# lucasnewman/f5-tts-mlx

Measured on AMD Instinct MI355X. Metric: mel_frames_per_sec, higher is better.
Workload: dtype f16 (IEEE-half MFMA operands, fp32 accumulate / residual stream / LayerNorm / softmax state; meets the 1e-3 gate); 1 GPU; BASELINE configs[1]: F5-TTS 335M, 32-point euler (=62 DiT forwards, CFG), batch 1/GPU x 10 s (N=937) utterances, hipGraph=True; f16 (IEEE half) MFMA operands IN PLACE OF BASELINE's bf16 -- same width and MFMA rate, three more significand bits; plain bf16 fails the 1e-3 parity gate, see sub.b1_bf16; global_batch=1, seq_len=937, parallelism=dp1 (utterance sharding)

## Files before the change

### f5_tts_mlx_amd/csrc/gemm.hip

```cpp
#include "gemm.hpp"
#include "gemm_dev.hpp"
#include "rowops.hpp"
#include "lnrow.hpp"

namespace F5_NS {



template <int MB, int NB>
struct ResidPre {
    float x[MB][16][NB];
    float bias[NB], gate[NB];
    uint32_t keep[MB][4];
};
template <int MB, int NB>
__device__ __forceinline__ void resid_preload(const F5GemmArgs& p, ResidPre<MB, NB>& q, int row0, int colbase, int lane) {
    const int hi = lane >> 5, lcol = lane & 31;
    const bool keep_words = p.rowkeep != nullptr && (reinterpret_cast<uintptr_t>(p.rowkeep) & 3) == 0;
#pragma unroll
    for (int nb = 0; nb < NB; ++nb) {
        const int c = colbase + nb * 32 + lcol;
        const bool ok = c < p.N;
        q.bias[nb] = (p.bias != nullptr && ok) ? p.bias[c] : 0.0f;
        q.gate[nb] = ok ? p.gate[c] : 0.0f;
// ... 198 lines not shown
        pa[ks] = &smem[0][0] + swz_off(wm * (32 * MB) + frow, ks * 2 + fk);
        pb[ks] = &smem[0][0] + BMt * BK + swz_off(wn * (32 * NB) + frow, ks * 2 + fk);
    }
    static_assert(2 * (BMt + BNt) * BK * 2 <= 65536, "both buffers must be addressable by ds_read immediates");
#define REG_STEP(CUR, tt_)                                                                                    \
    {                                                                                                         \
        if ((tt_) + 1 < T) LOAD_TILE();                                                                       \
        _Pragma("unroll") for (int ks = 0; ks < 4; ++ks) {                                                    \
            op16x8 af[MB], bfr[NB];                                                                           \
            _Pragma("unroll") for (int mb = 0; mb < MB; ++mb)                                                 \
                af[mb] = *reinterpret_cast<const op16x8*>(pa[ks] + (CUR) * (BMt + BNt) * BK + mb * 32 * BK);  \
            _Pragma("unroll") for (int nb = 0; nb < NB; ++nb)                                                 \
                bfr[nb] = *reinterpret_cast<const op16x8*>(pb[ks] + (CUR) * (BMt + BNt) * BK + nb * 32 * BK); \
            _Pragma("unroll") for (int mb = 0; mb < MB; ++mb)                                                 \
                _Pragma("unroll") for (int nb = 0; nb < NB; ++nb)                                             \
                    acc[mb][nb] = F5_MFMA32(af[mb], bfr[nb], acc[mb][nb], 0, 0, 0); \
        }                                                                                                     \
        if ((tt_) + 1 < T) STORE_TILE(1 - (CUR));                                                             \
        __syncthreads();                                                                                      \
    }
    for (int tt = 0; tt < T; tt += 2) {
        REG_STEP(0, tt);
        if (tt + 1 < T) REG_STEP(1, tt + 1);
    }
#undef REG_STEP
#undef LOAD_TILE
#undef STORE_TILE

    if (small_tile_staged<EPI, NB>() && n0 + BNt <= p.N && (p.debug_flags & 2) == 0) {
        static_assert(!small_tile_staged<EPI, NB>() || 4 * small_tile_stage_elems<NB>() <= 2 * (BMt + BNt) * BK, "staging fits");
        __syncthreads();
        staged_epilogue_bf16<EPI, MB, NB>(p, acc, &smem[0][0] + wave * small_tile_stage_elems<NB>(), m0 + wm * (32 * MB),
                                          n0 + wn * (32 * NB), lane);
        return;
    }
    gemm_epilogue<EPI, MB, NB>(p, acc, m0, n0, wm, wn, lane);
    if (EPI == EPI_RESID_GATE && p.ln_counter) resid_ln_tail(p, tm, BMt, (p.N + BNt - 1) / BNt);
}

int f5_gemm_order = 0;
static bool gemm_mfast(const F5GemmArgs& a) {
    if (f5_gemm_order == 1) return false;
    if (f5_gemm_order == 2) return true;
    const size_t a_bytes = (size_t)(a.a_row_mod > 0 ? a.a_row_mod : a.M) * a.K * 2 * (a.nseg == 3 ? 2 : 1);
    return a_bytes <= (size_t)4 << 20;
}
static int ring_order(const F5GemmArgs& a, int tiles_m, int tiles_n) {
    const bool band_ok = tiles_n % 4 == 0 && tiles_n >= 8 && (long)tiles_m * tiles_n <= 512 && tiles_m >= 8;
    if ((f5_gemm_order == 3 || f5_gemm_order == 0) && band_ok) return tiles_n | (4 << 20);
    if (f5_gemm_order == 3) return tiles_n;
    return gemm_mfast(a) ? -tiles_m : tiles_n;
}

template <int EPI, int MB, int NB, int NST, int WM = 2, int WN = 2, int KS = 1, int ABL = 0, int FOLD = 0>
__global__ __launch_bounds__(64 * WM * WN * KS) void f5_gemm_ring_kernel(F5GemmArgs p, int tiles_n, int ntiles) {
    constexpr int NTG = 64 * WM * WN;
    constexpr int BMt = 32 * MB * WM, BNt = 32 * NB * WN;
    constexpr int NA = BMt * 8 / NTG, NW = BNt * 8 / NTG;
    static_assert(NA * NTG == BMt * 8 && NW * NTG == BNt * 8, "tile rows must divide over the threads");
    constexpr int G = NA + NW;
    constexpr int STAGE = (BMt + BNt) * BK;
    constexpr int RING = NST * STAGE;
    static_assert(KS * RING * 2 <= 160 * 1024, "LDS budget");
    __shared__ __attribute__((aligned(16))) op16_t smem_all[KS * RING];

    asm volatile("" ::"s"(p.A[0]), "s"(p.W[0]), "s"(p.lda), "s"(p.ldw), "s"(p.K), "s"(p.nseg), "s"(p.M), "s"(p.N), "s"(p.a_row_mod),
                 "s"(p.debug_flags), "s"(tiles_n), "s"(ntiles));
    if (EPI == EPI_RESID_GATE)
        asm volatile("" ::"s"(p.bias), "s"(p.out_f32), "s"(p.ldo), "s"(p.gate), "s"(p.rowkeep), "s"(p.ln_counter));
    const int bid = blockIdx.x;
    const int q = ntiles >> 3, r = ntiles & 7;
    const int xcd = bid & 7, idx = bid >> 3;
    const int tile = (xcd < r ? xcd * (q + 1) : r * (q + 1) + (xcd - r) * q) + idx;
    int tm, tn;
    if (tiles_n >= (1 << 20)) {
        const int band = tiles_n >> 20, tnn = tiles_n & ((1 << 20) - 1);
        const int per_band = band * (ntiles / tnn);
        const int b = tile / per_band, rem = tile - b * per_band;
        tm = rem / band;
        tn = b * band + (rem - tm * band);
    } else if (tiles_n > 0) {
        tm = tile / tiles_n;
        tn = tile - tm * tiles_n;
    } else {
        tn = tile / (-tiles_n);
        tm = tile - tn * (-tiles_n);
    }
    const int m0 = tm * BMt, n0 = tn * BNt;

    const int tid = threadIdx.x;
    const int lane = tid & 63;
    const int wave_all = __builtin_amdgcn_readfirstlane(tid >> 6);
    const int grp = wave_all / (WM * WN), wave = wave_all % (WM * WN);
    const int tg = tid - grp * NTG;
    const int wm = wave / WN, wn = wave % WN;
    op16_t* smem = smem_all + grp * RING;

    uint32_t a_src[NA], w_src[NW];
    int a_dst[NA], w_dst[NW];
#pragma unroll
    for (int i = 0; i < NA; ++i) {
        const int q_ = i * NTG + tg;
        const int row = q_ >> 3, chunk = (q_ & 7) ^ ((row >> 1) & 7);
        int gr = m0 + row;
        if (gr > p.M - 1) gr = p.M - 1;
        if (p.a_row_mod > 0) gr = gr % p.a_row_mod;
        a_src[i] = ((uint32_t)gr * (uint32_t)p.lda + chunk * 8) * 2u;
        a_dst[i] = (i * NTG + wave * 64) * 8;
    }
#pragma unroll
    for (int i = 0; i < NW; ++i) {
        const int q_ = i * NTG + tg;
        const int row = q_ >> 3, chunk = (q_ & 7) ^ ((row >> 1) & 7);
        w_src[i] = ((uint32_t)(n0 + row) * (uint32_t)p.ldw + chunk * 8) * 2u;
        w_dst[i] = BMt * BK + (i * NTG + wave * 64) * 8;
    }
    const int kt = p.K / BK;
    const int T = kt * p.nseg;
    const int Tg = T > grp ? (T - grp + KS - 1) / KS : 0;
    const int nit = (T + KS - 1) / KS;
    int is_seg = 0, is_k0 = grp * BK;
    while (is_k0 >= p.K) {
        is_k0 -= p.K;
        ++is_seg;
    }
#define RING_ISSUE(ST_)                                                                                      \
    {                                                                                                        \
        op16_t* st_ = smem + (ST_) * STAGE;                                                                  \
        const char* Ap_ = reinterpret_cast<const char*>((is_seg == 1) ? p.A[1] : p.A[0]);                    \
        const char* Wp_ = reinterpret_cast<const char*>((is_seg == 2) ? p.W[1] : p.W[0]);                    \
        const uint32_t kb_ = (uint32_t)is_k0 * 2u;                                                           \
        _Pragma("unroll") for (int i = 0; i < NA; ++i)                                                       \
            glds16(reinterpret_cast<const op16_t*>(Ap_ + (a_src[i] + kb_)), st_ + a_dst[i]);                 \
        _Pragma("unroll") for (int i = 0; i < NW; ++i)                                                       \
            glds16(reinterpret_cast<const op16_t*>(Wp_ + (w_src[i] + kb_)), st_ + w_dst[i]);                 \
        is_k0 += KS * BK;                                                                                    \
        while (is_k0 >= p.K) {                                          \
            is_k0 -= p.K;                                                                                    \
            ++is_seg;                                                                                        \
        }                                                                                                    \
    }

    f32x16 acc[MB][NB];
#pragma unroll
    for (int i = 0; i < MB; ++i)
#pragma unroll
        for (int j = 0; j < NB; ++j)
#pragma unroll
            for (int e = 0; e < 16; ++e) acc[i][j][e] = 0.0f;

    constexpr bool PRE_RESID = EPI == EPI_RESID_GATE && MB * NB <= 3;
    ResidPre<PRE_RESID ? MB : 1, PRE_RESID ? NB : 1> rpre;
    const bool use_pre = PRE_RESID && p.ln_counter == nullptr && (p.debug_flags & (8 | 256)) == 0;
    constexpr bool SHARE = KS > 1 && NB == KS && FOLD == 0 && EPI != EPI_QKV_ROPE;
    const bool share = SHARE && p.ln_counter == nullptr && (p.debug_flags & (8 | 256)) == 0;
    constexpr bool SHARE_PRE = SHARE && PRE_RESID;
    ResidPre<SHARE_PRE ? MB : 1, 1> rown;
    if constexpr (SHARE_PRE) {
        if (use_pre) resid_preload<MB, 1>(p, rown, m0 + wm * (32 * MB), n0 + wn * (32 * NB) + grp * 32, lane);
    }
    if (PRE_RESID && !SHARE_PRE && use_pre && grp == 0 && FOLD != 1)
        resid_preload<PRE_RESID ? MB : 1, PRE_RESID ? NB : 1>(p, rpre, m0 + wm * (32 * MB), n0 + wn * (32 * NB), lane);
    static_assert(FOLD == 0 || (FOLD == 1 && PRE_RESID && NB == 2) || (FOLD == 2 && EPI == EPI_GELU_TANH && NB == 2 && KS == 1 && WM * WN == 8),
                  "fold producer = the preloaded residual epilogue on 64-column wave tiles; fold consumer = the 8-wave GELU launch");
    ResidStagedPre<FOLD == 1 ? NB : 1> spre_p;
    if constexpr (FOLD == 1) {
        if (grp == 0) resid_staged_preload<NB>(p, spre_p, m0 + wm * (32 * MB), n0 + wn * (32 * NB), lane);
    }
    FoldPre fpre_c;
    fold_prefetch_clear(fpre_c);
    FoldStatsPre<8> spre_c;
    fold_stats_clear(spre_c);
    if constexpr (FOLD == 2) fold_stats_request_tr<1>(p, spre_c, fpre_c, m0 + wm * 32, n0 + wn * 64, lane);

#pragma unroll
    for (int st = 0; st < NST - 1; ++st)
        if (st < Tg) RING_ISSUE(st);

    const int frow = lane & 31;
    const int fk = lane >> 5;
    constexpr int SPS = 65536 / (STAGE * 2) < NST ? 65536 / (STAGE * 2) : NST;
    static_assert(SPS >= 1, "a stage must fit the ds_read offset field");
    constexpr int NSET = (NST + SPS - 1) / SPS;
    const op16_t* pa[NSET][4];
    const op16_t* pb[NSET][4];
#pragma unroll
    for (int w2 = 0; w2 < NSET; ++w2)
#pragma unroll
        for (int ks = 0; ks < 4; ++ks) {
            pa[w2][ks] = smem + w2 * SPS * STAGE + swz_off(wm * (32 * MB) + frow, ks * 2 + fk);
            pb[w2][ks] = smem + w2 * SPS * STAGE + BMt * BK + swz_off(wn * (32 * NB) + frow, ks * 2 + fk);
        }
    op16x8 abl_frag;
#pragma unroll
    for (int e = 0; e < 8; ++e) abl_frag[e] = (op16_t)0;
    if (ABL & 4) asm volatile("" : "+v"(abl_frag));
#define RING_STEP(ST_, jj_, TR_)                                                                                       \
    {                                                                                                               \
         \
        if ((jj_) + NST - 2 < Tg) {                                                                                 \
            if (NST == 4) asm volatile("s_waitcnt vmcnt(%0)" ::"n"(2 * G) : "memory");                              \
            else if (NST == 3) asm volatile("s_waitcnt vmcnt(%0)" ::"n"(G) : "memory");                             \
            else asm volatile("s_waitcnt vmcnt(0)" ::: "memory");                                                   \
        } else {                                                                                                    \
            asm volatile("s_waitcnt vmcnt(0)" ::: "memory");                                                        \
        }                                                                                                           \
        asm volatile("" ::: "memory");                                                                              \
        if (!(ABL & 8)) __builtin_amdgcn_s_barrier();                                                               \
        asm volatile("" ::: "memory");                                                                              \
        if (!(ABL & 1) && (jj_) + NST - 1 < Tg) RING_ISSUE(((ST_) + NST - 1) % NST);  \
        if (!(KS > 1 && (jj_) >= Tg)) {               \
            constexpr int W2 = (ST_) / SPS, SL = (ST_) % SPS;                                                        \
            _Pragma("unroll") for (int ks = 0; ks < 4; ++ks) {                                                      \
                op16x8 af[MB], bfr[NB];                                                                             \
                _Pragma("unroll") for (int mb = 0; mb < MB; ++mb)                                                   \
                    af[mb] = (ABL & 4) ? abl_frag : *reinterpret_cast<const op16x8*>(pa[W2][ks] + SL * STAGE + mb * 32 * BK); \
                _Pragma("unroll") for (int nb = 0; nb < NB; ++nb)                                                   \
                    bfr[nb] = (ABL & 4) ? abl_frag : *reinterpret_cast<const op16x8*>(pb[W2][ks] + SL * STAGE + nb * 32 * BK); \
                _Pragma("unroll") for (int mb = 0; mb < MB; ++mb)                                                   \
                    _Pragma("unroll") for (int nb = 0; nb < NB; ++nb) {                                             \
                        if (ABL & 2) asm volatile("" ::"v"(af[mb]), "v"(bfr[nb]));                                  \
                        else if (TR_) acc[mb][nb] = F5_MFMA32(bfr[nb], af[mb], acc[mb][nb], 0, 0, 0);               \
                        else acc[mb][nb] = F5_MFMA32(af[mb], bfr[nb], acc[mb][nb], 0, 0, 0);                        \
                    }                                                                                               \
            }                                                                                                       \
        }                                                                                                           \
    }
    if constexpr (FOLD == 2) {
        if (NST == 4) asm volatile("s_waitcnt vmcnt(%0)" ::"n"(2 * G) : "memory");
        else asm volatile("s_waitcnt vmcnt(0)" ::: "memory");
        fold_stats_pin(spre_c);
        fold_stats_finish_tr<1>(p, spre_c, fpre_c, m0 + wm * 32, lane, p.fold_mean_out != nullptr && n0 == 0 && wn == 0);
        fold_prefetch_pin(fpre_c);
        for (int jj = 0; jj < nit; jj += NST) {
            RING_STEP(0, jj, true);
            if (NST > 1 && jj + 1 < nit) RING_STEP(1 % NST, jj + 1, true);
            if (NST > 2 && jj + 2 < nit) RING_STEP(2 % NST, jj + 2, true);
            if (NST > 3 && jj + 3 < nit) RING_STEP(3 % NST, jj + 3, true);
        }
        __syncthreads();
        static_assert(FOLD != 2 || WM * WN * (small_tile_stage_elems<NB>() * 2 + 512) <= RING * 2, "staging + c1 | c2 scratch fit in the ring");
        float* fl = reinterpret_cast<float*>(smem_all + WM * WN * small_tile_stage_elems<NB>()) + wave * 128;
        staged_epilogue_tr<EPI, MB, NB, true>(p, acc, smem_all + wave * small_tile_stage_elems<NB>(), m0 + wm * (32 * MB), n0 + wn * (32 * NB), lane,
                                              fl, &fpre_c);
        return;
    }
    constexpr bool QKV_TR_OK = EPI == EPI_QKV_ROPE && (32 * NB) % 64 == 0 && (NB & (NB - 1)) == 0 && KS == 1 && WM * WN == 8;
    if (QKV_TR_OK && p.rope_g4k != nullptr && n0 + wn * (32 * NB) < 2 * p.dmodel) {
        for (int jj = 0; jj < nit; jj += NST) {
            RING_STEP(0, jj, true);
            if (NST > 1 && jj + 1 < nit) RING_STEP(1 % NST, jj + 1, true);
            if (NST > 2 && jj + 2 < nit) RING_STEP(2 % NST, jj + 2, true);
            if (NST > 3 && jj + 3 < nit) RING_STEP(3 % NST, jj + 3, true);
        }
        __syncthreads();
        staged_epilogue_tr_rope<MB, NB>(p, acc, smem_all + wave * small_tile_stage_elems<NB>(), m0 + wm * (32 * MB), n0 + wn * (32 * NB),
                                        lane);
        return;
    }
    for (int jj = 0; jj < nit; jj += NST) {
        RING_STEP(0, jj, false);
        if (NST > 1 && jj + 1 < nit) RING_STEP(1 % NST, jj + 1, false);
        if (NST > 2 && jj + 2 < nit) RING_STEP(2 % NST, jj + 2, false);
        if (NST > 3 && jj + 3 < nit) RING_STEP(3 % NST, jj + 3, false);
    }
#undef RING_STEP
#undef RING_ISSUE
    if constexpr (SHARE) {
        if (share) {
            constexpr int RED1 = MB * 16 * 64;
            constexpr int STG1 = small_tile_staged<EPI, 1>() ? small_tile_stage_elems<1>() : 0;
            constexpr int STGS = KS * WM * WN * STG1;
            static_assert(STGS * 2 + WM * WN * NB * (KS - 1) * RED1 * 4 <= KS * RING * 2, "staging + parked parts fit in the rings");
            float* red = reinterpret_cast<float*>(smem_all + STGS) + (size_t)wave * (NB * (KS - 1) * RED1) + lane;
            __syncthreads();
#pragma unroll
            for (int g = 0; g < KS; ++g)
                if (grp == g) {
#pragma unroll
                    for (int nb = 0; nb < NB; ++nb)
                        if (nb != g) {
                            float* dst = red + (nb * (KS - 1) + (g < nb ? g : g - 1)) * RED1;
#pragma unroll
                            for (int mb = 0; mb < MB; ++mb)
#pragma unroll
                                for (int e = 0; e < 16; ++e) dst[(mb * 16 + e) * 64] = acc[mb][nb][e];
                        }
                }
            __syncthreads();
            f32x16 own[MB][1];
#pragma unroll
            for (int g = 0; g < KS; ++g)
                if (grp == g) {
                    const float* src = red + g * (KS - 1) * RED1;
#pragma unroll
                    for (int mb = 0; mb < MB; ++mb)
#pragma unroll
                        for (int e = 0; e < 16; ++e) {
                            const float mine = acc[mb][g][e];
                            float s = g == 0 ? mine : src[(mb * 16 + e) * 64];
#pragma unroll
                            for (int h = 1; h < KS; ++h) s += h == g ? mine : src[(h < g ? h : h - 1) * RED1 + (mb * 16 + e) * 64];
                            own[mb][0][e] = s;
                        }
                }
            const int row0 = m0 + wm * (32 * MB), col0 = n0 + wn * (32 * NB) + grp * 32;
            if (small_tile_staged<EPI, NB>() && n0 + BNt <= p.N && (p.debug_flags & 2) == 0) {
                staged_epilogue_bf16<EPI, MB, 1>(p, own, smem_all + wave_all * STG1, row0, col0, lane);
                return;
            }
            if constexpr (SHARE_PRE) {
                if (use_pre) {
                    resid_epilogue_preloaded<MB, 1>(p, own, rown, row0, col0, lane);
                    return;
                }
            }
            gemm_epilogue<EPI, MB, 1>(p, own, m0, col0, wm, 0, lane);
            return;
        }
    }
    constexpr int STG = small_tile_staged<EPI, NB>() ? WM * WN * small_tile_stage_elems<NB>() : 0;
    if (KS > 1) {
        constexpr int RED = MB * NB * 16 * 64;
        static_assert(KS == 1 || STG * 2 + (KS - 1) * WM * WN * RED * 4 <= KS * RING * 2, "reduction area fits in the rings");
        float* red = reinterpret_cast<float*>(smem_all + STG);
        __syncthreads();
        if (grp > 0) {
            float* dst = red + (size_t)((grp - 1) * (WM * WN) + wave) * RED + lane;
#pragma unroll
            for (int mb = 0; mb < MB; ++mb)
#pragma unroll
                for (int nb = 0; nb < NB; ++nb)
#pragma unroll
                    for (int e = 0; e < 16; ++e) dst[((mb * NB + nb) * 16 + e) * 64] = acc[mb][nb][e];
        }
        __syncthreads();
        if (grp > 0) {
            if (EPI == EPI_RESID_GATE && p.ln_counter) resid_ln_tail(p, tm, BMt, (p.N + BNt - 1) / BNt);
            return;
        }
#pragma unroll
        for (int g = 1; g < KS; ++g) {
            const float* src = red + (size_t)((g - 1) * (WM * WN) + wave) * RED + lane;
#pragma unroll
            for (int mb = 0; mb < MB; ++mb)
#pragma unroll
                for (int nb = 0; nb < NB; ++nb)
#pragma unroll
                    for (int e = 0; e < 16; ++e) acc[mb][nb][e] += src[((mb * NB + nb) * 16 + e) * 64];
        }
    }
    if (small_tile_staged<EPI, NB>() && n0 + BNt <= p.N && (p.debug_flags & 2) == 0) {
        static_assert(STG <= RING, "staging fits");
        if (KS == 1) __syncthreads();
        staged_epilogue_bf16<EPI, MB, NB>(p, acc, smem_all + wave * small_tile_stage_elems<NB>(), m0 + wm * (32 * MB),
                                          n0 + wn * (32 * NB), lane);
        return;
    }
    if constexpr (FOLD == 1) {
        constexpr int RED_BYTES = (KS - 1) * WM * WN * MB * NB * 16 * 64 * 4;
        static_assert(RED_BYTES + WM * WN * 32 * (32 * NB + 4) * 4 <= KS * RING * 2, "staging behind the reduction area");
        float* stg = reinterpret_cast<float*>(reinterpret_cast<char*>(smem_all) + RED_BYTES) + wave * (32 * (32 * NB + 4));
        staged_epilogue_resid<MB, NB, true>(p, acc, stg, m0 + wm * (32 * MB), n0 + wn * (32 * NB), lane, &spre_p);
        return;
    }
    if constexpr (PRE_RESID) {
        if (use_pre) {
            resid_epilogue_preloaded<MB, NB>(p, acc, rpre, m0 + wm * (32 * MB), n0 + wn * (32 * NB), lane);
            return;
        }
    }
    gemm_epilogue<EPI, MB, NB>(p, acc, m0, n0, wm, wn, lane);
    if (EPI == EPI_RESID_GATE && p.ln_counter) resid_ln_tail(p, tm, BMt, (p.N + BNt - 1) / BNt);
}

template <int EPI, int MB, int NB, int NST, int WM = 2, int WN = 2, int KS = 1, int FOLD = 0>
static int launch_ring(const F5GemmArgs& a, hipStream_t stream) {
    const int tiles_m = f5_cdiv(a.M, 32 * MB * WM), tiles_n = f5_cdiv(a.N, 32 * NB * WN);
    const int ntiles = tiles_m * tiles_n;
    const int order = ring_order(a, tiles_m, tiles_n);
    hipLaunchKernelGGL((f5_gemm_ring_kernel<EPI, MB, NB, NST, WM, WN, KS, 0, FOLD>), dim3(ntiles), dim3(64 * WM * WN * KS), 0, stream, a, order, ntiles);
    F5_LAUNCH_CHECK();
    return 0;
}

template <int EPI, int MB, int NB>
static int launch_cfg(const F5GemmArgs& a, hipStream_t stream) {
    const int tiles_m = f5_cdiv(a.M, 64 * MB), tiles_n = f5_cdiv(a.N, 64 * NB);
    const int ntiles = tiles_m * tiles_n;
    hipLaunchKernelGGL((f5_gemm_kernel<EPI, MB, NB>), dim3(ntiles), dim3(256), 0, stream, a, tiles_n, ntiles);
    F5_LAUNCH_CHECK();
    return 0;
}

int f5_gemm_debug_flags = 0;

constexpr int FC_ROWS = 4, FC_MAXC = 8;
int f5_fold_consts_mfma = 1;
__global__ __launch_bounds__(256) void f5_fold_consts_kernel(const op16_t* __restrict__ w, int ldw, const float* __restrict__ bias,
                                                             const float* __restrict__ scale, const float* __restrict__ shift, size_t vec_stride,
                                                             int nvec, float* __restrict__ c1, float* __restrict__ c2, size_t out_stride, int N,
                                                             int K, F5FoldBatch bt) {
    w += (size_t)blockIdx.y * bt.w_stride;
    if (bias) bias += (size_t)blockIdx.y * bt.bias_stride;
    scale += (size_t)blockIdx.y * bt.mod_stride;
    shift += (size_t)blockIdx.y * bt.mod_stride;
    c1 += (size_t)blockIdx.y * bt.out_blk_stride;
    c2 += (size_t)blockIdx.y * bt.out_blk_stride;
    const int lane = threadIdx.x & 63, wave = threadIdx.x >> 6;
    const int n0 = (blockIdx.x * 4 + wave) * FC_ROWS;
    if (n0 >= N) return;
    const int nchunk = K >> 8;
    float wv[FC_ROWS][FC_MAXC][4];
#pragma unroll
    for (int r = 0; r < FC_ROWS; ++r) {
        const int n = n0 + r < N ? n0 + r : N - 1;
#pragma unroll
        for (int c = 0; c < FC_MAXC; ++c) {
            if (c < nchunk) {
                const op16x4 t = *reinterpret_cast<const op16x4*>(w + (size_t)n * ldw + c * 256 + lane * 4);
#pragma unroll
                for (int e = 0; e < 4; ++e) wv[r][c][e] = f5_op2f(t[e]);
            } else {
#pragma unroll
                for (int e = 0; e < 4; ++e) wv[r][c][e] = 0.0f;
            }
        }
    }
    for (int v = 0; v < nvec; ++v) {
        const float* sv = scale + (size_t)v * vec_stride;
        const float* bv = shift + (size_t)v * vec_stride;
        float a1[FC_ROWS], a2[FC_ROWS];
#pragma unroll
        for (int r = 0; r < FC_ROWS; ++r) a1[r] = a2[r] = 0.0f;
#pragma unroll
        for (int c = 0; c < FC_MAXC; ++c) {
            if (c < nchunk) {
                const f32x4 s4 = *reinterpret_cast<const f32x4*>(sv + c * 256 + lane * 4);
                const f32x4 b4 = *reinterpret_cast<const f32x4*>(bv + c * 256 + lane * 4);
#pragma unroll
                for (int r = 0; r < FC_ROWS; ++r)
#pragma unroll
                    for (int e = 0; e < 4; ++e) {
                        a1[r] += wv[r][c][e] * (1.0f + s4[e]);
                        a2[r] += wv[r][c][e] * b4[e];
                    }
            }
        }
#pragma unroll
        for (int r = 0; r < FC_ROWS; ++r) {
            a1[r] = f5_wave_sum(a1[r]);
            a2[r] = f5_wave_sum(a2[r]);
        }
        if (lane == 0) {
#pragma unroll
            for (int r = 0; r < FC_ROWS; ++r)
                if (n0 + r < N) {
                    c1[(size_t)v * out_stride + n0 + r] = a1[r];
                    c2[(size_t)v * out_stride + n0 + r] = a2[r] + (bias ? bias[n0 + r] : 0.0f);
                }
        }
    }
}

template <int NVB>
__global__ __launch_bounds__(256) void f5_fold_consts_mfma_kernel(const op16_t* __restrict__ w, int ldw, const float* __restrict__ bias,
                                                                  const float* __restrict__ scale, const float* __restrict__ shift,
                                                                  size_t vec_stride, int nvec, float* __restrict__ c1, float* __restrict__ c2,
                                                                  size_t out_stride, int N, int K, F5FoldBatch bt) {
    w += (size_t)blockIdx.y * bt.w_stride;
    if (bias) bias += (size_t)blockIdx.y * bt.bias_stride;
    scale += (size_t)blockIdx.y * bt.mod_stride;
    shift += (size_t)blockIdx.y * bt.mod_stride;
    c1 += (size_t)blockIdx.y * bt.out_blk_stride;
    c2 += (size_t)blockIdx.y * bt.out_blk_stride;
    const int lane = threadIdx.x & 63, wave = threadIdx.x >> 6;
    const int n0 = (blockIdx.x * 4 + wave) * 32;
    if (n0 >= N) return;
    const int lr = lane & 31, kh = (lane >> 5) * 8;
    const int nrow = n0 + lr < N ? n0 + lr : N - 1;
    const op16_t* wp = w + (size_t)nrow * ldw + kh;
    const float* sp[NVB];
    const float* bp[NVB];
#pragma unroll
    for (int vb = 0; vb < NVB; ++vb) {
        const int v = vb * 32 + lr < nvec ? vb * 32 + lr : nvec - 1;
        sp[vb] = scale + (size_t)v * vec_stride + kh;
        bp[vb] = shift + (size_t)v * vec_stride + kh;
    }
    f32x16 a1[NVB], a2[NVB];
#pragma unroll
    for (int vb = 0; vb < NVB; ++vb)
#pragma unroll
        for (int e = 0; e < 16; ++e) a1[vb][e] = a2[vb][e] = 0.0f;
    auto split = [](const f32x4& lo4, const f32x4& hi4, float add, op16x8& h, op16x8& l) {
#pragma unroll
        for (int e = 0; e < 8; ++e) {
            const float f = (e < 4 ? lo4[e] : hi4[e - 4]) + add;
            const op16_t hh = f5_f2op(f);
            h[e] = hh;
            l[e] = static_cast<op16_t>(f - static_cast<float>(hh));
        }
    };
    for (int k0 = 0; k0 < K; k0 += 16) {
        const op16x8 wf = *reinterpret_cast<const op16x8*>(wp + k0);
#pragma unroll
        for (int vb = 0; vb < NVB; ++vb) {
            const f32x4 s0 = *reinterpret_cast<const f32x4*>(sp[vb] + k0), s1 = *reinterpret_cast<const f32x4*>(sp[vb] + k0 + 4);
            const f32x4 b0 = *reinterpret_cast<const f32x4*>(bp[vb] + k0), b1 = *reinterpret_cast<const f32x4*>(bp[vb] + k0 + 4);
            op16x8 sh, sl, bh, bl;
            split(s0, s1, 1.0f, sh, sl);
            split(b0, b1, 0.0f, bh, bl);
            a1[vb] = F5_MFMA32(sh, wf, a1[vb], 0, 0, 0);
            a1[vb] = F5_MFMA32(sl, wf, a1[vb], 0, 0, 0);
            a2[vb] = F5_MFMA32(bh, wf, a2[vb], 0, 0, 0);
            a2[vb] = F5_MFMA32(bl, wf, a2[vb], 0, 0, 0);
// ... 198 lines not shown
```

### f5_tts_mlx_amd/csrc/gemm_dev.hpp

```cpp
#pragma once
#include "gemm.hpp"

namespace F5_NS {

#define BK 64

__device__ __forceinline__ f5_f32x2 f5_bc2(float s) {
    asm volatile("" : "+v"(s));
    return f5_f32x2{s, s};
}
__device__ __forceinline__ f5_f32x2 f5_fma2(f5_f32x2 a, f5_f32x2 b, f5_f32x2 c) { return __builtin_elementwise_fma(a, b, c); }

__device__ __forceinline__ int swz_off(int row, int chunk) {
    return row * BK + ((chunk ^ ((row >> 1) & 7)) << 3);
}

template <int EPI, int MB, int NB>
__device__ __forceinline__ void gemm_epilogue(const F5GemmArgs& p, f32x16 (&acc)[MB][NB], int m0, int n0, int wm, int wn,
                                               int lane) {
    const int hi = lane >> 5;
    const int lcol = lane & 31;
    f5_sat_t trk;
    int col[NB];
    bool colok[NB];
// ... 506 lines not shown
            }
    }
#pragma unroll
    for (int mb = 0; mb < MBW; ++mb) {
        const int rowblk = row0 + mb * 32;
        f5_f32x2 rr = {1.0f, 0.0f};
        if (FOLD) rr = rrv[mb];
        const f5_f32x2 r0v = f5_bc2(rr[0]), nr1v = f5_bc2(-rr[1]);
#pragma unroll
        for (int nb = 0; nb < NBW; ++nb)
#pragma unroll
            for (int rg = 0; rg < 4; ++rg) {
                const f32x4 c1q = FOLD ? c1r[nb][rg] : f32x4{0.f, 0.f, 0.f, 0.f}, c2q = b4[nb][rg];
                f5_f32x2 v[2];
#pragma unroll
                for (int h = 0; h < 2; ++h) {
                    const f5_f32x2 a = {acc[mb][nb][rg * 4 + 2 * h], acc[mb][nb][rg * 4 + 2 * h + 1]};
                    const f5_f32x2 c2h = {c2q[2 * h], c2q[2 * h + 1]};
                    if (FOLD) {
                        const f5_f32x2 c1h = {c1q[2 * h], c1q[2 * h + 1]};
                        v[h] = f5_fma2(r0v, a, f5_fma2(nr1v, c1h, c2h));
                    } else {
                        v[h] = a + c2h;
                    }
                    if (EPI == EPI_GELU_TANH) v[h] = f5_gelu_tanh2(v[h]);
                    if (EPI == EPI_GELU_ERF_BF16) v[h] = f5_f32x2{f5_gelu_erf(v[h][0]), f5_gelu_erf(v[h][1])};
                }
                const int so = lcol * LD + nb * 32 + rg * 8 + hi * 4;
                *reinterpret_cast<u32x2*>(&rh[so]) = u32x2{f5_pack2(v[0][0], v[0][1], trk), f5_pack2(v[1][0], v[1][1], trk)};
                if (two) *reinterpret_cast<u32x2*>(&rl[so]) = u32x2{f5_pack2_lo(v[0][0], v[0][1]), f5_pack2_lo(v[1][0], v[1][1])};
            }
        __builtin_amdgcn_wave_barrier();
        u32x4 back[32 / RPI];
#pragma unroll
        for (int i = 0; i < 32 / RPI; ++i) back[i] = *reinterpret_cast<const u32x4*>(&rh[(i * RPI + lane / CPR) * LD + (lane % CPR) * 8]);
#pragma unroll
        for (int i = 0; i < 32 / RPI; ++i) asm volatile("" : "+v"(back[i]));
#pragma unroll
        for (int i = 0; i < 32 / RPI; ++i) {
            const int lrow = i * RPI + lane / CPR, chunk = lane % CPR;
            const int grow = rowblk + lrow;
            if (grow < p.M) {
                const size_t off = (size_t)grow * p.ldob + colbase + chunk * 8;
                *reinterpret_cast<u32x4*>(p.out_bf[0] + off) = back[i];
                if (two) *reinterpret_cast<u32x4*>(p.out_bf[1] + off) = *reinterpret_cast<const u32x4*>(&rl[lrow * LD + chunk * 8]);
            }
        }
        __builtin_amdgcn_wave_barrier();
    }
    f5_sat_commit(trk, p.sat_flag);
}

template <int MBW, int NBW, bool FOLD = false>
__device__ __forceinline__ void staged_epilogue_tr_rope(const F5GemmArgs& p, f32x16 (&acc)[MBW][NBW], op16_t* reg, int row0,
                                                        int colbase, int lane, float* fl = nullptr, const FoldPre* pre = nullptr) {
    constexpr int W = 32 * NBW;
    constexpr int LD = W + 8;
    constexpr int CPR = W / 8;
    constexpr int RPI = 64 / CPR;
    const int hi = lane >> 5, lcol = lane & 31;
    const bool two = p.out_bf[1] != nullptr;
    const bool isq = colbase < p.dmodel;
    typedef __attribute__((address_space(1))) const char gcchar;
    typedef __attribute__((address_space(1))) const f32x4 gcf32x4;
    gcchar* const tb = (gcchar*)(isq ? p.rope_g4q : p.rope_g4k);
    const uint32_t gstep = (uint32_t)p.seq_len * 16u;
    op16_t* rh = reg;
    op16_t* rl = reg + 32 * LD;
    f5_sat_t trk;
    f5_f32x2 rrv[MBW];
    if (FOLD) {
        static_assert(!FOLD || W == 64, "one column of c1 | c2 per lane");
#pragma unroll
        for (int mb = 0; mb < MBW; ++mb) rrv[mb] = pre->rr[mb];
        fl[lane] = pre->c[0];
        fl[W + lane] = pre->c[1];
        __builtin_amdgcn_wave_barrier();
    }
#pragma unroll
    for (int mb = 0; mb < MBW; ++mb) {
        const int rowblk = row0 + mb * 32;
        int row = rowblk + lcol;
        if (row > p.M - 1) row = p.M - 1;
        const int n = row % p.seq_len;
        uint32_t loff = (uint32_t)(hi * p.seq_len + n) * 16u;
        f5_f32x2 rr = {1.0f, 0.0f};
        if (FOLD) rr = rrv[mb];
        const f5_f32x2 nr1v = f5_bc2(-rr[1]);
#pragma unroll
        for (int nb = 0; nb < NBW; ++nb) {
            float c0[4], c1[4], s0[4], s1[4];
            f32x4 b4[4];
#pragma unroll
            for (int rg = 0; rg < 4; ++rg) {
                const int c = colbase + nb * 32 + rg * 8 + hi * 4;
                const int g0 = (((colbase & 63) + nb * 32 + rg * 8) & 63) >> 2;
                gcchar* gb = tb + (size_t)g0 * gstep;
                asm volatile("" : "+v"(loff));
                const f32x4 cs = *(gcf32x4*)(gb + loff);
                c0[rg] = cs[0];
                c1[rg] = cs[1];
                s0[rg] = cs[2];
                s1[rg] = cs[3];
                if (FOLD) {
                    const f32x4 c1q = *reinterpret_cast<const f32x4*>(&fl[c - colbase]), c2q = *reinterpret_cast<const f32x4*>(&fl[W + c - colbase]);
                    const f5_f32x2 lo = f5_fma2(nr1v, f5_f32x2{c1q[0], c1q[1]}, f5_f32x2{c2q[0], c2q[1]});
                    const f5_f32x2 hi2 = f5_fma2(nr1v, f5_f32x2{c1q[2], c1q[3]}, f5_f32x2{c2q[2], c2q[3]});
                    b4[rg] = f32x4{lo[0], lo[1], hi2[0], hi2[1]};
                } else {
                    b4[rg] = p.bias ? *reinterpret_cast<const f32x4*>(p.bias + c) : f32x4{0.f, 0.f, 0.f, 0.f};
                }
            }
            const f5_f32x2 rsv = f5_bc2(FOLD ? rr[0] : 1.0f);
#pragma unroll
            for (int rg = 0; rg < 4; ++rg) {
                f5_f32x2 a01 = {acc[mb][nb][rg * 4 + 0], acc[mb][nb][rg * 4 + 1]}, a23 = {acc[mb][nb][rg * 4 + 2], acc[mb][nb][rg * 4 + 3]};
                const f5_f32x2 b01 = {b4[rg][0], b4[rg][1]}, b23 = {b4[rg][2], b4[rg][3]};
                if (FOLD) {
                    a01 = f5_fma2(rsv, a01, b01);
                    a23 = f5_fma2(rsv, a23, b23);
                } else {
                    a01 = a01 + b01;
                    a23 = a23 + b23;
                }
                const f5_f32x2 t01 = a01 * f5_bc2(c0[rg]), t23 = a23 * f5_bc2(c1[rg]);
                const float o0 = __builtin_fmaf(-a01[1], s0[rg], t01[0]), o1 = __builtin_fmaf(a01[0], s0[rg], t01[1]);
                const float o2 = __builtin_fmaf(-a23[1], s1[rg], t23[0]), o3 = __builtin_fmaf(a23[0], s1[rg], t23[1]);
                const int so = lcol * LD + nb * 32 + rg * 8 + hi * 4;
                *reinterpret_cast<u32x2*>(&rh[so]) = u32x2{f5_pack2(o0, o1, trk), f5_pack2(o2, o3, trk)};
                if (two) *reinterpret_cast<u32x2*>(&rl[so]) = u32x2{f5_pack2_lo(o0, o1), f5_pack2_lo(o2, o3)};
            }
        }
        __builtin_amdgcn_wave_barrier();
        u32x4 back[32 / RPI];
#pragma unroll
        for (int i = 0; i < 32 / RPI; ++i) back[i] = *reinterpret_cast<const u32x4*>(&rh[(i * RPI + lane / CPR) * LD + (lane % CPR) * 8]);
#pragma unroll
        for (int i = 0; i < 32 / RPI; ++i) asm volatile("" : "+v"(back[i]));
#pragma unroll
        for (int i = 0; i < 32 / RPI; ++i) {
            const int lrow = i * RPI + lane / CPR, chunk = lane % CPR;
            const int grow = rowblk + lrow;
            if (grow < p.M) {
                const size_t off = (size_t)grow * p.ldob + colbase + chunk * 8;
                *reinterpret_cast<u32x4*>(p.out_bf[0] + off) = back[i];
                if (two) *reinterpret_cast<u32x4*>(p.out_bf[1] + off) = *reinterpret_cast<const u32x4*>(&rl[lrow * LD + chunk * 8]);
            }
        }
        __builtin_amdgcn_wave_barrier();
    }
    f5_sat_commit(trk, p.sat_flag);
}

template <int NBW>
struct ResidStagedPre {
    f32x4 xr[32 / (64 / (32 * NBW / 4))];
    uint32_t kraw[32 / (64 / (32 * NBW / 4))];
    float xsh[32 / (64 / (32 * NBW / 4))];
    float bcol[NBW];
    f32x4 g4, sc4;
};
template <int NBW>
__device__ __forceinline__ void resid_staged_preload(const F5GemmArgs& p, ResidStagedPre<NBW>& q, int row0, int colbase, int lane) {
    constexpr int CPR = 32 * NBW / 4, RPI = 64 / CPR, NI = 32 / RPI;
    const int chunk = lane % CPR;
#pragma unroll
    for (int i = 0; i < NI; ++i) {
        const int grow = row0 + i * RPI + lane / CPR;
        const bool ok = grow < p.M;
        q.xr[i] = ok ? *reinterpret_cast<const f32x4*>(p.out_f32 + (size_t)grow * p.ldo + colbase + chunk * 4) : f32x4{0.f, 0.f, 0.f, 0.f};
        q.kraw[i] = (ok && p.rowkeep != nullptr) ? (uint32_t)p.rowkeep[grow] : 1u;
        q.xsh[i] = (ok && p.x16_out != nullptr && p.x16_shift != nullptr) ? p.x16_shift[grow] : 0.0f;
    }
#pragma unroll
    for (int nb = 0; nb < NBW; ++nb) q.bcol[nb] = p.bias ? p.bias[colbase + nb * 32 + (lane & 31)] : 0.0f;
    q.g4 = *reinterpret_cast<const f32x4*>(p.gate + colbase + chunk * 4);
    q.sc4 = f32x4{1.0f, 1.0f, 1.0f, 1.0f};
    if (p.x16_out != nullptr) {
        const f32x4 t = *reinterpret_cast<const f32x4*>(p.x16_scale + colbase + chunk * 4);
#pragma unroll
        for (int e = 0; e < 4; ++e) q.sc4[e] += t[e];
    }
}
template <int MBW, int NBW, bool PRE = false>
__device__ __forceinline__ void staged_epilogue_resid(const F5GemmArgs& p, f32x16 (&acc)[MBW][NBW], float* reg, int row0,
                                                      int colbase, int lane, const ResidStagedPre<NBW>* pre = nullptr) {
    static_assert(!PRE || MBW == 1, "the preloaded form covers one 32-row block");
    constexpr int W = 32 * NBW;
    constexpr int LD = W + 4;
    constexpr int CPR = W / 4;
    constexpr int RPI = 64 / CPR;
    constexpr int NI = 32 / RPI;
    const int hi = lane >> 5, lcol = lane & 31;
    float bcol[NBW];
#pragma unroll
    for (int nb = 0; nb < NBW; ++nb) bcol[nb] = PRE ? pre->bcol[nb] : (p.bias ? p.bias[colbase + nb * 32 + lcol] : 0.0f);
    const int chunk = lane % CPR;
    f32x4 g4 = PRE ? pre->g4 : *reinterpret_cast<const f32x4*>(p.gate + colbase + chunk * 4);
    asm volatile("" : "+v"(g4));
    f32x4 sc4 = {1.0f, 1.0f, 1.0f, 1.0f};
    if (PRE) {
        sc4 = pre->sc4;
    } else if (p.x16_out != nullptr) {
        const f32x4 t = *reinterpret_cast<const f32x4*>(p.x16_scale + colbase + chunk * 4);
#pragma unroll
        for (int e = 0; e < 4; ++e) sc4[e] += t[e];
    }
#pragma unroll
    for (int mb = 0; mb < MBW; ++mb) {
        const int rowblk = row0 + mb * 32;
        f32x4 xr[NI];
        float xsh[NI];
        uint32_t kraw[NI];
#pragma unroll
        for (int i = 0; i < NI; ++i) {
            if (PRE) {
                xr[i] = pre->xr[i];
                kraw[i] = pre->kraw[i];
                xsh[i] = pre->xsh[i];
                continue;
            }
            const int grow = rowblk + i * RPI + lane / CPR;
            const bool ok = grow < p.M;
            xr[i] = ok ? *reinterpret_cast<const f32x4*>(p.out_f32 + (size_t)grow * p.ldo + colbase + chunk * 4)
                       : f32x4{0.f, 0.f, 0.f, 0.f};
            kraw[i] = (ok && p.rowkeep != nullptr) ? (uint32_t)p.rowkeep[grow] : 1u;
            xsh[i] = (CPR == 16 && ok && p.x16_out != nullptr && p.x16_shift != nullptr) ? p.x16_shift[grow] : 0.0f;
        }
#pragma unroll
        for (int r = 0; r < 16; ++r) {
            const int lrow = (r & 3) + 8 * (r >> 2) + 4 * hi;
#pragma unroll
            for (int nb = 0; nb < NBW; ++nb) reg[lrow * LD + nb * 32 + lcol] = acc[mb][nb][r] + bcol[nb];
        }
#pragma unroll
        for (int i = 0; i < NI; ++i) asm volatile("" : "+v"(xr[i]), "+v"(kraw[i]), "+v"(xsh[i]));
        __builtin_amdgcn_wave_barrier();
#pragma unroll
        for (int i = 0; i < NI; ++i) {
            const int lrow = i * RPI + lane / CPR;
            const int grow = rowblk + lrow;
            const f32x4 v = *reinterpret_cast<const f32x4*>(&reg[lrow * LD + chunk * 4]);
            f32x4 o;
#pragma unroll
            for (int e = 0; e < 4; ++e) o[e] = xr[i][e] + g4[e] * (kraw[i] != 0u ? v[e] : 0.0f);
            if (grow < p.M) *reinterpret_cast<f32x4*>(p.out_f32 + (size_t)grow * p.ldo + colbase + chunk * 4) = o;
            if (CPR == 16 && p.x16_out != nullptr) {
                const bool rok = grow < p.M;
                float d[4];
#pragma unroll
                for (int e = 0; e < 4; ++e) d[e] = rok ? o[e] - xsh[i] : 0.0f;
                float ps = (d[0] + d[1]) + (d[2] + d[3]);
                ps += f5_dpp_row<0x128>(ps);
                ps += f5_dpp_row<0x124>(ps);
                ps += f5_dpp_row<0x122>(ps);
                ps += f5_dpp_row<0x121>(ps);
                const float ms = ps * (1.0f / 64.0f);
                const float e0 = d[0] - ms, e1 = d[1] - ms, e2 = d[2] - ms, e3 = d[3] - ms;
                float pq = rok ? (e0 * e0 + e1 * e1) + (e2 * e2 + e3 * e3) : 0.0f;
                pq += f5_dpp_row<0x128>(pq);
                pq += f5_dpp_row<0x124>(pq);
                pq += f5_dpp_row<0x122>(pq);
                pq += f5_dpp_row<0x121>(pq);
#if F5_F16
                if (p.x16_overflow != nullptr) {
                    const bool ov = rok && !(fmaxf(fmaxf(fabsf(d[0] * sc4[0]), fabsf(d[1] * sc4[1])),
                                                   fmaxf(fabsf(d[2] * sc4[2]), fabsf(d[3] * sc4[3]))) <= 65504.0f);
                    if (__any(ov) && lane == 0) atomicOr(p.x16_overflow, 1);
                }
#endif
                if (rok) {
                    *reinterpret_cast<u32x2*>(p.x16_out + (size_t)grow * p.ldx16 + colbase + chunk * 4) =
                        u32x2{f5_pack2(d[0] * sc4[0], d[1] * sc4[1]), f5_pack2(d[2] * sc4[2], d[3] * sc4[3])};
                    if (chunk == 0)
                        *reinterpret_cast<f5_f32x2*>(p.stats_out + ((size_t)(colbase >> 6) * p.stats_ld + grow) * 2) = f5_f32x2{ps, pq};
                }
            }
        }
        __builtin_amdgcn_wave_barrier();
    }
}

__device__ __forceinline__ const char* v2_uniform_ptr(const void* ptr) {
    const uint64_t u = reinterpret_cast<uint64_t>(ptr);
    const uint32_t lo = __builtin_amdgcn_readfirstlane((uint32_t)u), hi = __builtin_amdgcn_readfirstlane((uint32_t)(u >> 32));
    return reinterpret_cast<const char*>(((uint64_t)hi << 32) | lo);
}

}
```

Baseline: 13880 mel-frames/s.

## Run fold-producer residual epilogue on split-K shared halves with merged row statistics

```diff
diff --git a/f5_tts_mlx_amd/csrc/gemm.hip b/f5_tts_mlx_amd/csrc/gemm.hip
--- a/f5_tts_mlx_amd/csrc/gemm.hip
+++ b/f5_tts_mlx_amd/csrc/gemm.hip
@@ -374,21 +374,20 @@
     constexpr bool PRE_RESID = EPI == EPI_RESID_GATE && MB * NB <= 3;
     ResidPre<PRE_RESID ? MB : 1, PRE_RESID ? NB : 1> rpre;
     const bool use_pre = PRE_RESID && p.ln_counter == nullptr && (p.debug_flags & (8 | 256)) == 0;
-    constexpr bool SHARE = KS > 1 && NB == KS && FOLD == 0 && EPI != EPI_QKV_ROPE;
-    const bool share = SHARE && p.ln_counter == nullptr && (p.debug_flags & (8 | 256)) == 0;
-    constexpr bool SHARE_PRE = SHARE && PRE_RESID;
+    constexpr bool SHARE = KS > 1 && NB == KS && EPI != EPI_QKV_ROPE;
+    const bool share = SHARE && (FOLD == 1 || (p.ln_counter == nullptr && (p.debug_flags & (8 | 256)) == 0));
+    constexpr bool SHARE_PRE = SHARE && PRE_RESID && FOLD != 1;
     ResidPre<SHARE_PRE ? MB : 1, 1> rown;
     if constexpr (SHARE_PRE) {
         if (use_pre) resid_preload<MB, 1>(p, rown, m0 + wm * (32 * MB), n0 + wn * (32 * NB) + grp * 32, lane);
     }
-    if (PRE_RESID && !SHARE_PRE && use_pre && grp == 0 && FOLD != 1)
+    if (PRE_RESID && !SHARE && use_pre && grp == 0)
         resid_preload<PRE_RESID ? MB : 1, PRE_RESID ? NB : 1>(p, rpre, m0 + wm * (32 * MB), n0 + wn * (32 * NB), lane);
-    static_assert(FOLD == 0 || (FOLD == 1 && PRE_RESID && NB == 2) || (FOLD == 2 && EPI == EPI_GELU_TANH && NB == 2 && KS == 1 && WM * WN == 8),
-                  "fold producer = the preloaded residual epilogue on 64-column wave tiles; fold consumer = the 8-wave GELU launch");
-    ResidStagedPre<FOLD == 1 ? NB : 1> spre_p;
-    if constexpr (FOLD == 1) {
-        if (grp == 0) resid_staged_preload<NB>(p, spre_p, m0 + wm * (32 * MB), n0 + wn * (32 * NB), lane);
-    }
+    static_assert(FOLD == 0 || (FOLD == 1 && PRE_RESID && SHARE && MB == 1 && KS == 2) ||
+                      (FOLD == 2 && EPI == EPI_GELU_TANH && NB == 2 && KS == 1 && WM * WN == 8),
+                  "fold producer = the preloaded residual epilogue on the halves of 64-column wave tiles; fold consumer = the 8-wave GELU launch");
+    ResidStagedPre<1> spre_p;
+    if constexpr (FOLD == 1) resid_staged_preload<1>(p, spre_p, m0 + wm * (32 * MB), n0 + wn * (32 * NB) + grp * 32, lane);
     FoldPre fpre_c;
     fold_prefetch_clear(fpre_c);
     FoldStatsPre<8> spre_c;
@@ -527,7 +526,25 @@
                         }
                 }
             const int row0 = m0 + wm * (32 * MB), col0 = n0 + wn * (32 * NB) + grp * 32;
-            if (small_tile_staged<EPI, NB>() && n0 + BNt <= p.N && (p.debug_flags & 2) == 0) {
+            if constexpr (FOLD == 1) {
+                constexpr int PARK = STGS * 2 + WM * WN * NB * (KS - 1) * RED1 * 4;
+                constexpr int STGF = 32 * (32 + 4), NWAVE = KS * WM * WN;
+                static_assert(PARK + NWAVE * (STGF + 64) * 4 <= KS * RING * 2, "staging + statistics pairs behind the parked parts fit in the rings");
+                float* stg = reinterpret_cast<float*>(reinterpret_cast<char*>(smem_all) + PARK);
+                float* pairs = stg + NWAVE * STGF;
+                staged_epilogue_resid<1, 1, true>(p, own, stg + wave_all * STGF, row0, col0, lane, &spre_p, pairs + wave_all * 64);
+                __syncthreads();
+                if (lane < 16 && p.x16_out != nullptr) {
+                    const int lrow = grp * 16 + lane, grow = row0 + lrow;
+                    const f5_f32x2 h0 = *reinterpret_cast<const f5_f32x2*>(pairs + wave * 64 + lrow * 2);
+                    const f5_f32x2 h1 = *reinterpret_cast<const f5_f32x2*>(pairs + (WM * WN + wave) * 64 + lrow * 2);
+                    if (grow < p.M)
+                        *reinterpret_cast<f5_f32x2*>(p.stats_out + ((size_t)((n0 + wn * (32 * NB)) >> 6) * p.stats_ld + grow) * 2) =
+                            fold_merge_halves(h0, h1);
+                }
+                return;
+            }
+            if (small_tile_staged<EPI, NB>()&& n0 + BNt <= p.N && (p.debug_flags & 2) == 0) {
                 staged_epilogue_bf16<EPI, MB, 1>(p, own, smem_all + wave_all * STG1, row0, col0, lane);
                 return;
             }
@@ -577,13 +594,6 @@
         if (KS == 1) __syncthreads();
         staged_epilogue_bf16<EPI, MB, NB>(p, acc, smem_all + wave * small_tile_stage_elems<NB>(), m0 + wm * (32 * MB),
                                           n0 + wn * (32 * NB), lane);
-        return;
-    }
-    if constexpr (FOLD == 1) {
-        constexpr int RED_BYTES = (KS - 1) * WM * WN * MB * NB * 16 * 64 * 4;
-        static_assert(RED_BYTES + WM * WN * 32 * (32 * NB + 4) * 4 <= KS * RING * 2, "staging behind the reduction area");
-        float* stg = reinterpret_cast<float*>(reinterpret_cast<char*>(smem_all) + RED_BYTES) + wave * (32 * (32 * NB + 4));
-        staged_epilogue_resid<MB, NB, true>(p, acc, stg, m0 + wm * (32 * MB), n0 + wn * (32 * NB), lane, &spre_p);
         return;
     }
     if constexpr (PRE_RESID) {
diff --git a/f5_tts_mlx_amd/csrc/gemm_dev.hpp b/f5_tts_mlx_amd/csrc/gemm_dev.hpp
--- a/f5_tts_mlx_amd/csrc/gemm_dev.hpp
+++ b/f5_tts_mlx_amd/csrc/gemm_dev.hpp
@@ -682,6 +682,17 @@
     f5_sat_commit(trk, p.sat_flag);
 }
 
+__device__ __forceinline__ float f5_row8_sum(float v) {
+    v += f5_dpp_row<0xB1>(v);
+    v += f5_dpp_row<0x4E>(v);
+    v += f5_dpp_row<0x141>(v);
+    return v;
+}
+__device__ __forceinline__ f5_f32x2 fold_merge_halves(f5_f32x2 h0, f5_f32x2 h1) {
+    const float dl = h0[0] - h1[0];
+    return f5_f32x2{h0[0] + h1[0], (h0[1] + h1[1]) + dl * dl * (1.0f / 64.0f)};
+}
+
 template <int NBW>
 struct ResidStagedPre {
     f32x4 xr[32 / (64 / (32 * NBW / 4))];
@@ -714,8 +725,10 @@
 }
 template <int MBW, int NBW, bool PRE = false>
 __device__ __forceinline__ void staged_epilogue_resid(const F5GemmArgs& p, f32x16 (&acc)[MBW][NBW], float* reg, int row0,
-                                                      int colbase, int lane, const ResidStagedPre<NBW>* pre = nullptr) {
+                                                      int colbase, int lane, const ResidStagedPre<NBW>* pre = nullptr,
+                                                      float* half_stats = nullptr) {
     static_assert(!PRE || MBW == 1, "the preloaded form covers one 32-row block");
+    constexpr bool HALF = PRE && NBW == 1;
     constexpr int W = 32 * NBW;
     constexpr int LD = W + 4;
     constexpr int CPR = W / 4;
@@ -775,23 +788,29 @@
 #pragma unroll
             for (int e = 0; e < 4; ++e) o[e] = xr[i][e] + g4[e] * (kraw[i] != 0u ? v[e] : 0.0f);
             if (grow < p.M) *reinterpret_cast<f32x4*>(p.out_f32 + (size_t)grow * p.ldo + colbase + chunk * 4) = o;
-            if (CPR == 16 && p.x16_out != nullptr) {
+            if ((CPR == 16 || HALF) && p.x16_out != nullptr) {
                 const bool rok = grow < p.M;
                 float d[4];
 #pragma unroll
                 for (int e = 0; e < 4; ++e) d[e] = rok ? o[e] - xsh[i] : 0.0f;
                 float ps = (d[0] + d[1]) + (d[2] + d[3]);
-                ps += f5_dpp_row<0x128>(ps);
-                ps += f5_dpp_row<0x124>(ps);
-                ps += f5_dpp_row<0x122>(ps);
-                ps += f5_dpp_row<0x121>(ps);
-                const float ms = ps * (1.0f / 64.0f);
+                if constexpr (HALF) ps = f5_row8_sum(ps);
+                else {
+                    ps += f5_dpp_row<0x128>(ps);
+                    ps += f5_dpp_row<0x124>(ps);
+                    ps += f5_dpp_row<0x122>(ps);
+                    ps += f5_dpp_row<0x121>(ps);
+                }
+                const float ms = ps * (1.0f / W);
                 const float e0 = d[0] - ms, e1 = d[1] - ms, e2 = d[2] - ms, e3 = d[3] - ms;
                 float pq = rok ? (e0 * e0 + e1 * e1) + (e2 * e2 + e3 * e3) : 0.0f;
-                pq += f5_dpp_row<0x128>(pq);
-                pq += f5_dpp_row<0x124>(pq);
-                pq += f5_dpp_row<0x122>(pq);
-                pq += f5_dpp_row<0x121>(pq);
+                if constexpr (HALF) pq = f5_row8_sum(pq);
+                else {
+                    pq += f5_dpp_row<0x128>(pq);
+                    pq += f5_dpp_row<0x124>(pq);
+                    pq += f5_dpp_row<0x122>(pq);
+                    pq += f5_dpp_row<0x121>(pq);
+                }
 #if F5_F16
                 if (p.x16_overflow != nullptr) {
                     const bool ov = rok && !(fmaxf(fmaxf(fabsf(d[0] * sc4[0]), fabsf(d[1] * sc4[1])),
@@ -802,9 +821,10 @@
                 if (rok) {
                     *reinterpret_cast<u32x2*>(p.x16_out + (size_t)grow * p.ldx16 + colbase + chunk * 4) =
                         u32x2{f5_pack2(d[0] * sc4[0], d[1] * sc4[1]), f5_pack2(d[2] * sc4[2], d[3] * sc4[3])};
-                    if (chunk == 0)
+                    if (!HALF && chunk == 0)
                         *reinterpret_cast<f5_f32x2*>(p.stats_out + ((size_t)(colbase >> 6) * p.stats_ld + grow) * 2) = f5_f32x2{ps, pq};
                 }
+                if (HALF && chunk == 0) *reinterpret_cast<f5_f32x2*>(half_stats + lrow * 2) = f5_f32x2{ps, pq};
             }
         }
         __builtin_amdgcn_wave_barrier();
```

Result: no change. 13830 mel-frames/s (-0.3%).
